# alexpreynolds/starch3

Hardware: AMD Instinct MI355X
Metric: input BED MB/s (cfg2, bzip2 -9, archive bit-identical to CPU starch3 path) (higher is better)
Workload: dtype u8

## Files before the change

starch_amd/csrc/bz2_bwt.hip:

```cpp
#include <string.h>
#include "bz2_int.hpp"
#include "bz2_bwt.hpp"

namespace bz {

constexpr int BT = 1024;
constexpr int NWV = BT / 64;

struct RadixSmem {
    uint32_t hist[256];
    uint32_t base[256];
    uint32_t wcnt[NWV][256];
    uint32_t scan[NWV + 1];
    uint32_t flag;
};

__device__ __forceinline__ uint64_t lanemask_lt()
{
    const int lane = threadIdx.x & 63;
    return lane ? (~0ull >> (64 - lane)) : 0ull;
}

template <class V>
__device__ bool radix_pass(const uint64_t* Ks, const V* Vs, uint64_t* Kd, V* Vd, uint32_t m, int shift,
// ... 713 lines not shown
                    slo[sp] = blo; shi[sp] = bhi; ++sp;
                }
                fbw_sync();
                continue;
            }
            const int32_t lo = cmd[1], hi = cmd[2], m = hi - lo + 1;
            for (int32_t q = lane; q < m; q += 64) { sk[q] = key[lo + q]; sf[q] = fmap[lo + q]; }
            __builtin_amdgcn_fence(__ATOMIC_RELEASE, "wavefront");
            __builtin_amdgcn_wave_barrier();
            __builtin_amdgcn_fence(__ATOMIC_ACQUIRE, "wavefront");
            if (lane == 0) fbp_qsort3(sk, sf, 0, m - 1, lcg);
            __builtin_amdgcn_fence(__ATOMIC_RELEASE, "wavefront");
            __builtin_amdgcn_wave_barrier();
            __builtin_amdgcn_fence(__ATOMIC_ACQUIRE, "wavefront");
            for (int32_t q = lane; q < m; q += 64) { key[lo + q] = sk[q]; fmap[lo + q] = sf[q]; }
            __builtin_amdgcn_fence(__ATOMIC_RELEASE, "wavefront");
            __builtin_amdgcn_wave_barrier();
            __builtin_amdgcn_fence(__ATOMIC_ACQUIRE, "wavefront");
        }
    }
}

__global__ void k_fb_heads(const uint32_t* __restrict__ key, const uint64_t* __restrict__ hp,
                           const uint32_t* __restrict__ mixed, uint32_t* __restrict__ head, uint32_t n, uint32_t stamp)
{
    const uint32_t i = blockIdx.x * blockDim.x + threadIdx.x;
    if (i == 0 || i >= n || head[i]) return;
    if (mixed[(uint32_t)hp[i]] == stamp && key[i] != key[i - 1]) head[i] = 1;
}

__global__ void k_fb_origptr(const uint32_t* __restrict__ fmap, BlockDesc* __restrict__ blocks, uint32_t b, uint32_t n)
{
    const uint32_t i = blockIdx.x * blockDim.x + threadIdx.x;
    if (i < n && fmap[i] == 0) blocks[b].orig_ptr = i;
}

void launch_bwt(BlockDesc* blocks, uint32_t b0, uint32_t nb, const uint8_t* blkbytes, uint64_t stride,
                const BwtScratch& scr, unsigned long long* stats, hipStream_t st)
{
    hipLaunchKernelGGL(k_bwt, dim3(nb), dim3(BT), 0, st, blocks, b0, blkbytes, stride, scr, stats);
    HIP_CHECK(hipGetLastError());
}

void FbPool::init(int device)
{
    if (dev == device) return;
    if (dev >= 0) throw StarchError(-10, "FbPool: device changed");
    for (int i = 0; i < kStreams; ++i) HIP_CHECK(hipStreamCreateWithFlags(&st[i], hipStreamNonBlocking));
    for (int i = 0; i <= kStreams; ++i) HIP_CHECK(hipEventCreateWithFlags(&ev[i], hipEventDisableTiming));
    dev = device;
}

FbPool::~FbPool()
{
    for (int i = 0; i < kStreams; ++i)
        if (st[i]) { (void)hipStreamSynchronize(st[i]); (void)hipStreamDestroy(st[i]); }
    for (int i = 0; i <= kStreams; ++i)
        if (ev[i]) (void)hipEventDestroy(ev[i]);
}

void launch_fallback(BlockDesc* blocks, uint32_t b0, const uint32_t* which_host, const uint32_t* n_host,
                     uint32_t nwhich, const uint8_t* blkbytes, uint64_t stride, const BwtScratch& scr, FbPool& pool,
                     hipStream_t st)
{
    int dev = 0, ncu = 256;
    HIP_CHECK(hipGetDevice(&dev));
    hipDeviceProp_t prop;
// ... 104 lines not shown
```

starch_amd/csrc/bz2_bwt3.hip:

```cpp
#include "bz2_int.hpp"
#include "bz2_bwt.hpp"

#include <algorithm>
#include <type_traits>

namespace bz {
namespace {

constexpr int PT = 256;
constexpr int PTILE = 32768;
constexpr int PDIG = 12;
constexpr int PNB = 1 << PDIG;
constexpr int PNB_WIDE = 8192;
static_assert(PTILE <= 32768 && PNB_WIDE <= 8192, "k3_scatter_lds packs (digit << 15) | rotation-in-tile");
constexpr int MAXT = (900064 + PTILE - 1) / PTILE;
constexpr uint32_t W_MAX = 64, S1_MAX = 128, S_MAX = 256, M0_MAX = 512, M1_MAX = 1024, M2_MAX = 2048, M3_MAX = 4096;
#ifndef STARCH_L_MIN
#define STARCH_L_MIN 4096
#endif
constexpr uint32_t L_MIN = STARCH_L_MIN;
constexpr uint32_t GB_MIN = 16384;
constexpr uint32_t GB_MAXN = 8192;
constexpr uint32_t HG_MIN_PUSH = 32768;
constexpr uint32_t RBITS = 20;
// ... 259 lines not shown
    if (tid < 256) {
        uint32_t c = tid, below = 0;
        for (uint32_t j = 0; j < (c >> 5); ++j) below += __popc(bd.in_use[j]);
        below += __popc(bd.in_use[c >> 5] & ((1u << (c & 31)) - 1u));
        sym[c] = (uint8_t)below;
    }
    uint32_t nin = 0;
    for (int j = 0; j < 8; ++j) nin += __popc(bd.in_use[j]);
    *nin_out = nin;
}

__device__ __forceinline__ uint32_t wg_pop(const Ctx& c, const uint32_t* qs, uint32_t* job_sh, uint32_t x)
{
    if (threadIdx.x == 0) *job_sh = xq_pop(c.qhead, qs, x);
    __syncthreads();
    const uint32_t j = *job_sh;
    __syncthreads();
    return j;
}

__device__ __forceinline__ uint32_t wave_pop(const Ctx& c, const uint32_t* qs, uint32_t x)
{
    uint32_t j = 0;
    if ((threadIdx.x & 63) == 0) j = xq_pop(c.qhead, qs, x);
    return (uint32_t)__shfl((int)j, 0, 64);
}

__device__ __forceinline__ void load_qsizes_binned(const Ctx& c, uint32_t* qs)
{
    if (threadIdx.x < 8) qs[threadIdx.x] = c.qseg[threadIdx.x + 1] - c.qseg[threadIdx.x];
    __syncthreads();
}

__global__ void __launch_bounds__(256) k3_pss(Ctx c)
{
    __shared__ uint8_t sym[256];
    const uint32_t slot = blockIdx.y, b = c.b0 + slot;
    const uint32_t n = c.blocks[b].n;
    uint32_t nin;
    load_sym(c.blocks[b], sym, &nin);
    const uint32_t B = nin > 1 ? (uint32_t)bits_for3(nin - 1) : 1u;
    const uint32_t nw = (uint32_t)(((uint64_t)(n + 128) * B + 63) / 64 + 1);
    if (blockIdx.x == 0 && threadIdx.x == 0) {
        Geo g;
        g.B = B;
        g.D = 64 / B;
        g.KB = g.D * B;
        g.Dp = (64 - PDIG) / B;
        g.nin = nin;
        g.D1 = (c.nbins == PNB_WIDE && B == 5 && nin <= 20) ? 3u : 0u;
        g.SH = g.D1 ? 3 * B : PDIG;
        g.pad = 0;
        c.L.geo[slot] = g;
        c.blocks[b].n_in_use = nin;
    }
    __syncthreads();
    const uint32_t w = blockIdx.x * 256 + threadIdx.x;
    if (w >= nw) return;
    const uint8_t* blk = c.blkbytes + (uint64_t)b * c.stride;
    const uint64_t bit0 = (uint64_t)w * 64;
    const uint64_t j0 = bit0 / B, j1 = (bit0 + 63) / B;
    uint64_t word = 0;
    if (B == 4 && j1 < n) {
        const uint4 v = *reinterpret_cast<const uint4*>(blk + j0);
        const uint32_t q[4] = {v.x, v.y, v.z, v.w};
#pragma unroll
        for (int k = 0; k < 16; ++k) word = (word << 4) | sym[(q[k >> 2] >> (8 * (k & 3))) & 0xffu];
        c.scr.K[(uint64_t)slot * c.scr.stride + w] = word;
        return;
    }
    for (uint64_t j = j0; j <= j1; ++j) {
        const uint64_t s = sym[blk[j < n ? j : j % n]];
        const int sh = 64 - (int)B - (int)(j * B - bit0);
        word |= sh >= 0 ? (s << sh) : (s >> (-sh));
    }
    c.scr.K[(uint64_t)slot * c.scr.stride + w] = word;
}

__device__ __forceinline__ uint32_t* tile_hist(const Ctx& c, uint32_t slot)
{
    return reinterpret_cast<uint32_t*>(c.scr.K + (uint64_t)slot * c.scr.stride + pss_words(c.scr.stride));
}

template <int NB>
__global__ void __launch_bounds__(PT) k3_hist(Ctx c)
{
    __shared__ uint32_t cnt[NB];
    const uint32_t slot = blockIdx.y, b = c.b0 + slot, tile = blockIdx.x;
    const uint32_t n = c.blocks[b].n;
    const uint32_t t0 = tile * PTILE;
    if (t0 >= n) return;
    const Geo geo = c.L.geo[slot];
    const uint32_t B = geo.B;
    const uint64_t* pss = c.scr.K + (uint64_t)slot * c.scr.stride;
    for (int i = threadIdx.x; i < NB; i += PT) cnt[i] = 0;
    __syncthreads();
    const uint32_t e = n - t0 < (uint32_t)PTILE ? n - t0 : (uint32_t)PTILE;
    for (uint32_t k0 = threadIdx.x * 16u; k0 < e; k0 += PT * 16u) {
        const uint64_t bit0 = (uint64_t)(t0 + k0) * B;
        const uint64_t q0 = bit0 >> 6;
        const uint32_t p0 = (uint32_t)(bit0 & 63u);
        const uint64_t w[4] = {pss[q0], pss[q0 + 1], pss[q0 + 2], pss[q0 + 3]};
#pragma unroll
        for (int k = 0; k < 16; ++k) {
            const uint32_t bit = p0 + (uint32_t)k * B;
            const uint32_t ix = bit >> 6, p = bit & 63u;
            const uint64_t a = ix == 0 ? w[0] : ix == 1 ? w[1] : w[2];
            const uint64_t nx = ix == 0 ? w[1] : ix == 1 ? w[2] : w[3];
            const uint64_t v = (a << p) | ((nx >> 1) >> (63u - p));
            if (k0 + k < e) atomicAdd(&cnt[top_digit(v, geo)], 1u);
        }
    }
    __syncthreads();
    uint32_t* th = tile_hist(c, slot) + (uint64_t)tile * NB;
    for (int i = threadIdx.x; i < NB; i += PT) th[i] = cnt[i];
}

constexpr int ST = 1024;

template <int NB>
__global__ void __launch_bounds__(ST) k3_scan(Ctx c)
{
    constexpr int Q = NB / (4 * ST);
    __shared__ uint32_t scan_sh[ST / 64 + 1];
    __shared__ uint32_t cls_sh[16];
    const int tid = threadIdx.x;
    const uint32_t slot = blockIdx.x, b = c.b0 + slot;
    const uint32_t n = c.blocks[b].n;
    const uint32_t ntile = (n + PTILE - 1) / PTILE;
    uint4* th = reinterpret_cast<uint4*>(tile_hist(c, slot));
    uint4* tot = th + (uint64_t)MAXT * (NB / 4);
    uint4 a[Q];
#pragma unroll
    for (int j = 0; j < Q; ++j) a[j] = make_uint4(0, 0, 0, 0);
#pragma unroll 4
    for (uint32_t k = 0; k < ntile; ++k) {
#pragma unroll
        for (int j = 0; j < Q; ++j) {
            const uint4 x = th[(uint64_t)k * (NB / 4) + tid * Q + j];
            a[j].x += x.x; a[j].y += x.y; a[j].z += x.z; a[j].w += x.w;
        }
    }
    uint32_t sum = 0;
#pragma unroll
// ... 2394 lines not shown
            }
            if (n0) {
                bin(c.L.m0, n0, bout);
                hipLaunchKernelGGL((k3_sort_lds<4, 2, D>), gm0, dim3(256), 0, st, c, bout, nullptr);
            }
            if (n1) {
                bin(c.L.m1, n1, bout);
                hipLaunchKernelGGL((k3_sort_lds<4, 4, D>), gm1, dim3(256), 0, st, c, bout, nullptr);
            }
            if (ns) {
                bin(c.L.s, ns, bout);
                clear_h();
                hipLaunchKernelGGL((k3_sort_grp<1, 2, D>), gs, dim3(256), 0, st, c, bout, c.L.s);
                hipLaunchKernelGGL((k3_sort_lds<1, 2, D>), dim3(ncu / 2), dim3(256), 0, st, c, c.L.s, hard_n);
            }
            if (ns2) {
                bin(c.L.s2, ns2, bout);
                clear_h();
                hipLaunchKernelGGL((k3_sort_grp<1, 4, D>), gs2, dim3(256), 0, st, c, bout, c.L.s2);
                hipLaunchKernelGGL((k3_sort_lds<1, 4, D>), dim3(ncu / 2), dim3(256), 0, st, c, c.L.s2, hard_n);
            }
            if (nw) {
                bin(c.L.w, nw, bout);
                hipLaunchKernelGGL(k3_sort_w<D>, gw, dim3(256), 0, st, c, bout);
            }
        };
        if (c.keysrc) leaf(std::true_type{});
        else leaf(std::false_type{});
        HIP_CHECK(hipGetLastError());
        zero((0x3Full << C_W) | bit(C_M0));
    };

    {
        const uint32_t maxw = (uint32_t)pss_words(scr.stride);
        hipLaunchKernelGGL(k3_pss, dim3((maxw + 255) / 256, nb), dim3(256), 0, st, c);
        if (wide) {
            hipLaunchKernelGGL(k3_hist<PNB_WIDE>, dim3(MAXT, nb), dim3(PT), 0, st, c);
            hipLaunchKernelGGL(k3_scan<PNB_WIDE>, dim3(nb), dim3(ST), 0, st, c);
        } else {
            hipLaunchKernelGGL(k3_hist<PNB>, dim3(MAXT, nb), dim3(PT), 0, st, c);
            hipLaunchKernelGGL(k3_scan<PNB>, dim3(nb), dim3(ST), 0, st, c);
        }
        uint32_t* head;
        uint32_t* seg;
        next_q(head, seg);
        c.qhead = head;
        c.qseg = nullptr;
        const dim3 gsc((ncu + 7) / 8 * 8);
        c.sdig = 1;
        if (wide) hipLaunchKernelGGL(k3_scatter_lds<PNB_WIDE>, gsc, dim3(SCT), 0, st, c);
        else hipLaunchKernelGGL(k3_scatter_lds<PNB>, gsc, dim3(SCT), 0, st, c);
        HIP_CHECK(hipGetLastError());
    }
    sort_groups();
    c.sdig = 0;
    uint32_t rtext = 0;
    uint64_t prev_tied = ~0ull;
    bool done = false;
    for (;;) {
        read_ctr();
        const uint32_t nt = hctr[C_T0 + c.tsel];
        const uint64_t tied = hctr[C_TS0 + c.tsel];
        if (nt == 0) { done = true; break; }
        if (rtext == TEXT_ROUNDS || (rtext > 0 && 2 * tied > prev_tied)) break;
        prev_tied = tied;
        ++rtext;
        c.rtext = rtext;
        const uint32_t cur = c.tsel;
        c.tsel ^= 1u;
        zero(bit(C_T0 + c.tsel) | bit(C_TS0 + c.tsel));
        hipLaunchKernelGGL(k3_classify_text, dim3((nt + 256 * CT_IPT - 1) / (256 * CT_IPT)), dim3(256), 0, st, c,
                           c.L.t[cur], nt);
        HIP_CHECK(hipGetLastError());
// ... 37 lines not shown
```

starch_amd/csrc/bz2_mtf.hip:

```cpp
#include "bz2_bwt.hpp"

namespace bz {

constexpr int MT = 1024;
constexpr int NCH_BIG = 256;
constexpr uint32_t LINE = 128;

__device__ __forceinline__ uint32_t nsym_run(uint32_t z) { return z ? (31 - __clz(z + 1)) : 0; }

struct RunSum {
    uint32_t nz;
    uint32_t lz;
    uint32_t tz;
    uint32_t inner;
};

__device__ __forceinline__ RunSum run_compose(const RunSum& a, const RunSum& b)
{
    RunSum r;
    if (!a.nz) {
        r.nz = b.nz; r.lz = a.lz + b.lz; r.tz = b.tz; r.inner = b.inner;
    } else if (!b.nz) {
        r.nz = 1; r.lz = a.lz; r.tz = a.tz + b.lz; r.inner = a.inner;
    } else {
// ... 70 lines not shown
        }
        ++o;
    }
    __device__ __forceinline__ void flush()
    {
        const uint32_t k = o & 15u;
        if (!k) return;
        const uint32_t w = o - k, p = s > w ? s - w : 0u;
        const uint32_t sh = 8u * (16u - k);
        const uint64_t rl = sh >= 64 ? hi >> (sh - 64) : ((lo >> sh) | (sh ? hi << (64 - sh) : 0ull));
        const uint64_t rh = sh >= 64 ? 0ull : hi >> sh;
        store_range(w, p, k, rl, rh);
    }
};

__device__ __forceinline__ void put_run(Out8& out, uint32_t z)
{
    while (z) {
        const uint32_t d = ((z - 1) & 1u) ? 1u : 0u;
        out.put(d);
        z = (z - (d + 1)) >> 1;
    }
}

constexpr uint32_t MCS = 512;
constexpr int MCT = 256;
constexpr int MST = 1024;

struct NibP {
    using State = NibState;
    using List = uint64_t;
    static constexpr uint32_t LO = 1, HI = 16;
    static constexpr uint32_t SW = 2, LW = 1;
    static constexpr uint32_t IXB = 4;
#ifndef STARCH_NIB_SIX
#define STARCH_NIB_SIX 0
#endif
    static constexpr bool SIX = STARCH_NIB_SIX != 0;
    __device__ static State empty() { State r; r.list = 0; r.set = 0; r.cnt = 0; return r; }
    __device__ static void add(State& st, uint32_t s)
    {
        if (!((st.set >> s) & 1u)) { st.set |= 1u << s; st.list |= (uint64_t)s << (4 * st.cnt); ++st.cnt; }
    }
    __device__ static State compose(const State& c, const State& d) { return nib_compose(c, d); }
    __device__ static State identity(uint32_t nin)
    {
        State st;
        st.list = 0;
        for (uint32_t i = 0; i < nin; ++i) st.list |= (uint64_t)i << (4 * i);
        st.set = nin >= 32 ? ~0u : (1u << nin) - 1u;
        st.cnt = nin;
        return st;
    }
    __device__ static List list_of(const State& st) { return st.list; }
    __device__ static uint32_t mtf(List& L, uint32_t s) { return nib_mtf(L, s); }
};

struct ByteState {
    uint64_t w[4];
    uint32_t set;
    uint32_t cnt;
};
struct ByteList { uint64_t w[4]; };

template <int NW>
struct ByteP {
    static_assert(NW == 3 || NW == 4, "ByteP: 3 or 4 list words");
    using State = ByteState;
    using List = ByteList;
    static constexpr uint32_t LO = NW == 3 ? 17 : 25, HI = NW == 3 ? 24 : 30;
    static constexpr uint32_t SW = 5, LW = 4;
    static constexpr uint32_t IXB = 8;
#ifndef STARCH_BYTE_SIX
#define STARCH_BYTE_SIX 0
#endif
    static constexpr bool SIX = STARCH_BYTE_SIX != 0;
    __device__ static void put(uint64_t* w, uint32_t i, uint32_t s)
    {
        const uint32_t j = i >> 3, sh = 8 * (i & 7);
#pragma unroll
        for (uint32_t q = 0; q < 4; ++q)
            if (q == j) w[q] = (w[q] & ~(0xFFull << sh)) | ((uint64_t)s << sh);
    }
    __device__ static uint32_t get(const uint64_t* w, uint32_t i)
    {
        const uint32_t j = i >> 3;
        const uint64_t x = j == 0 ? w[0] : j == 1 ? w[1] : j == 2 ? w[2] : w[3];
        return (uint32_t)(x >> (8 * (i & 7))) & 0xFFu;
    }
    __device__ static State empty()
    {
        State r;
        r.w[0] = r.w[1] = r.w[2] = r.w[3] = ~0ull;
        r.set = 0;
        r.cnt = 0;
        return r;
    }
    __device__ static void add(State& st, uint32_t s)
    {
        if (!((st.set >> s) & 1u)) { st.set |= 1u << s; put(st.w, st.cnt, s); ++st.cnt; }
    }
    __device__ static State compose(const State& c, const State& d)
    {
        State r = d;
        for (uint32_t i = 0; i < c.cnt; ++i) {
            const uint32_t sym = get(c.w, i);
            if (!((d.set >> sym) & 1u)) { put(r.w, r.cnt, sym); ++r.cnt; }
        }
        r.set = c.set | d.set;
// ... 17 lines not shown
    {
        const uint64_t pat = (uint64_t)s * 0x0101010101010101ull;
        uint64_t z[4] = {0, 0, 0, 0};
#pragma unroll
        for (int j = 0; j < NW; ++j) {
            const uint64_t x = L.w[j] ^ pat;
            z[j] = (x - 0x0101010101010101ull) & ~x & 0x8080808080808080ull;
        }
        const uint32_t k = z[0] ? ((uint32_t)__builtin_ctzll(z[0]) >> 3)
                         : z[1] ? 8u + ((uint32_t)__builtin_ctzll(z[1]) >> 3)
                         : (NW == 3 || z[2]) ? 16u + ((uint32_t)__builtin_ctzll(z[2]) >> 3)
                                : 24u + ((uint32_t)__builtin_ctzll(z[3]) >> 3);
        const uint32_t jk = k >> 3, kb = k & 7u;
        const uint64_t m = kb == 7u ? ~0ull : ((1ull << (8u * kb + 8u)) - 1ull);
        uint64_t carry = s;
#pragma unroll
        for (uint32_t j = 0; j < (uint32_t)NW; ++j) {
            const uint64_t nv = (L.w[j] << 8) | carry;
            carry = L.w[j] >> 56;
            L.w[j] = j < jk ? nv : (j == jk ? ((nv & m) | (L.w[j] & ~m)) : L.w[j]);
        }
        return k;
    }
};

template <class P>
struct MtfScr {
    uint64_t* base;
    uint32_t C;
    __device__ typename P::State* st() const { return reinterpret_cast<typename P::State*>(base); }
    __device__ typename P::List* l0() const { return reinterpret_cast<typename P::List*>(base + (uint64_t)P::SW * C); }
    __device__ RunSum* rs() const { return reinterpret_cast<RunSum*>(base + (uint64_t)(P::SW + P::LW) * C); }
    __device__ uint2* zo() const { return reinterpret_cast<uint2*>(base + (uint64_t)(P::SW + P::LW + 2) * C); }
    __device__ uint8_t* ix() const { return reinterpret_cast<uint8_t*>(base + (uint64_t)(P::SW + P::LW + 3) * C); }
};

template <class P>
__device__ __forceinline__ MtfScr<P> mtf_scr(uint64_t* K, uint64_t kstride, uint32_t slot, uint32_t C)
{
    MtfScr<P> m;
    m.base = K + (uint64_t)slot * kstride;
    m.C = C;
    return m;
}

template <class P>
__device__ __forceinline__ bool mtf_mine(uint32_t nin) { return nin >= P::LO && nin <= P::HI; }

template <class F>
__device__ __forceinline__ void visit_chunk(const uint8_t* ll, uint32_t a, uint32_t e, F&& f)
{
    const uint4* q = reinterpret_cast<const uint4*>(ll + a);
    const uint32_t np = (e - a + 15) / 16;
    uint4 cur = q[0];
#pragma unroll 1
    for (uint32_t i = 0; i < np; ++i) {
        const uint4 nxt = q[i + 1 < np ? i + 1 : i];
        const uint32_t lim = e - a - 16 * i;
        if (lim >= 16) {
            auto all = [&](int, uint32_t s) { f(s); };
            piece<true>(cur, 0, all);
        } else {
            auto some = [&](int k, uint32_t s) { if ((uint32_t)k < lim) f(s); };
            piece<true>(cur, 0, some);
        }
        cur = nxt;
    }
}

template <class F>
__device__ __forceinline__ void visit_chunk_lines(const uint8_t* ll, uint32_t a, uint32_t e, F&& f)
{
    const uint32_t full = a + ((e - a) & ~(LINE - 1));
#pragma unroll 1
    for (uint32_t j0 = a; j0 < full; j0 += LINE) visit_line<true>(ll + j0, [&](int, uint32_t s) { f(s); });
    if (full < e) {
        const uint32_t lim = e - full;
        visit_line<true>(ll + full, [&](int k, uint32_t s) { if ((uint32_t)k < lim) f(s); });
    }
}

template <class P>
__global__ void __launch_bounds__(MCT) k_mtf_local(const BlockDesc* __restrict__ blocks, uint32_t b0,
                                                   const uint8_t* __restrict__ LL, uint64_t ll_stride,
                                                   uint64_t* __restrict__ K, uint64_t kstride, uint32_t C, uint32_t cs)
{
    const uint32_t slot = blockIdx.y, b = b0 + slot;
    const uint32_t n = blocks[b].n, nin = blocks[b].n_in_use;
    const uint32_t ch = blockIdx.x * MCT + threadIdx.x;
    const uint32_t a = ch * cs;
    if (!mtf_mine<P>(nin) || a >= n) return;
    const uint32_t e = a + cs < n ? a + cs : n;
    const uint8_t* ll = LL + (uint64_t)slot * ll_stride;
    typename P::State loc = P::empty();
    const uint32_t full = a + ((e - a) & ~(LINE - 1));
    auto add = [&](uint32_t s) { P::add(loc, s); };
    if (full < e) {
        const uint32_t lim = e - full;
        visit_line<false>(ll + full, [&](int k, uint32_t s) { if ((uint32_t)k < lim) add(s); });
    }
#pragma unroll 1
    for (uint32_t j0 = full; j0 > a && loc.cnt < nin;) {
        j0 -= LINE;
        visit_line<false>(ll + j0, [&](int, uint32_t s) { add(s); });
    }
    mtf_scr<P>(K, kstride, slot, C).st()[ch] = loc;
}

template <class P>
__global__ void __launch_bounds__(MST) k_mtf_scan_lists(const BlockDesc* __restrict__ blocks, uint32_t b0,
                                                        uint64_t* __restrict__ K, uint64_t kstride, uint32_t C,
                                                        uint32_t cs)
{
    __shared__ typename P::State sh[MST];
    const int tid = threadIdx.x;
    const uint32_t slot = blockIdx.x, b = b0 + slot;
    const uint32_t n = blocks[b].n, nin = blocks[b].n_in_use;
    if (!mtf_mine<P>(nin)) return;
    const uint32_t nch = (n + cs - 1) / cs;
    const uint32_t per = (nch + MST - 1) / MST;
    const MtfScr<P> ms = mtf_scr<P>(K, kstride, slot, C);
    const uint32_t c0 = tid * per;
    typename P::State agg = P::empty();
    for (uint32_t q = 0; q < per; ++q)
        if (c0 + q < nch) agg = P::compose(agg, ms.st()[c0 + q]);
    sh[tid] = agg;
    __syncthreads();
    for (int d = 1; d < MST; d <<= 1) {
        const typename P::State v = (tid >= d) ? P::compose(sh[tid - d], sh[tid]) : sh[tid];
        __syncthreads();
        sh[tid] = v;
        __syncthreads();
    }
    typename P::State st = P::identity(nin);
    if (tid) st = P::compose(st, sh[tid - 1]);
    for (uint32_t q = 0; q < per; ++q) {
        if (c0 + q >= nch) break;
        ms.l0()[c0 + q] = P::list_of(st);
        st = P::compose(st, ms.st()[c0 + q]);
    }
}

template <class P>
__global__ void __launch_bounds__(MCT) k_mtf_runs(const BlockDesc* __restrict__ blocks, uint32_t b0,
                                                  const uint8_t* __restrict__ LL, uint64_t ll_stride,
                                                  uint64_t* __restrict__ K, uint64_t kstride, uint32_t C, uint32_t cs)
{
    const uint32_t slot = blockIdx.y, b = b0 + slot;
    const uint32_t n = blocks[b].n, nin = blocks[b].n_in_use;
    const uint32_t ch = blockIdx.x * MCT + threadIdx.x;
    const uint32_t a = ch * cs;
    if (!mtf_mine<P>(nin) || a >= n) return;
    const uint32_t e = a + cs < n ? a + cs : n;
    const MtfScr<P> ms = mtf_scr<P>(K, kstride, slot, C);
    uint32_t z = 0, nz = 0, lz = 0, inner = 0;
    if constexpr (!P::SIX) {
        const uint8_t* ll = LL + (uint64_t)slot * ll_stride;
        uint32_t prev = a ? ll[a - 1] : 0u;
        visit_chunk_lines(ll, a, e, [&](uint32_t s) {
            const uint32_t nzf = s != prev ? 1u : 0u;
            prev = s;
            inner += (nzf & nz) ? 1u + (31u - __clz(z + 1u)) : 0u;
            lz = (nzf & (nz ^ 1u)) ? z : lz;
            nz |= nzf;
            z = nzf ? 0u : z + 1u;
        });
        RunSum r;
        r.nz = nz;
        r.lz = nz ? lz : z;
        r.tz = nz ? z : 0u;
        r.inner = inner;
        ms.rs()[ch] = r;
        return;
    }
    typename P::List L = ms.l0()[ch];
    uint8_t* ixp = ms.ix() + (uint64_t)a * P::IXB / 8;
    uint64_t lo = 0, hi = 0;
    uint32_t k16 = 0, piece_no = 0;
    visit_chunk(LL + (uint64_t)slot * ll_stride, a, e, [&](uint32_t s) {
        const uint32_t x = P::mtf(L, s);
        if constexpr (P::IXB == 4) {
            lo = (lo >> 4) | ((uint64_t)x << 60);
        } else {
            lo = (lo >> 8) | (hi << 56);
            hi = (hi >> 8) | ((uint64_t)x << 56);
        }
        if (P::SIX && ++k16 == 16) {
            if constexpr (P::IXB == 4) reinterpret_cast<uint64_t*>(ixp)[piece_no] = lo;
            else reinterpret_cast<uint4*>(ixp)[piece_no] = make_uint4((uint32_t)lo, (uint32_t)(lo >> 32),
                                                                      (uint32_t)hi, (uint32_t)(hi >> 32));
            k16 = 0;
            ++piece_no;
        }
        const uint32_t nzf = x != 0 ? 1u : 0u;
        inner += (nzf & nz) ? 1u + (31u - __clz(z + 1u)) : 0u;
        lz = (nzf & (nz ^ 1u)) ? z : lz;
        nz |= nzf;
        z = nzf ? 0u : z + 1u;
    });
    if (P::SIX && k16) {
        const uint32_t sh = (16 - k16) * P::IXB;
        if constexpr (P::IXB == 4) {
            reinterpret_cast<uint64_t*>(ixp)[piece_no] = lo >> sh;
        } else {
            const uint64_t l2 = sh >= 64 ? hi >> (sh - 64) : ((lo >> sh) | (hi << (64 - sh)));
            const uint64_t h2 = sh >= 64 ? 0 : hi >> sh;
            reinterpret_cast<uint4*>(ixp)[piece_no] = make_uint4((uint32_t)l2, (uint32_t)(l2 >> 32), (uint32_t)h2,
                                                                 (uint32_t)(h2 >> 32));
        }
    }
    RunSum r;
    r.nz = nz;
    r.lz = nz ? lz : z;
    r.tz = nz ? z : 0u;
    r.inner = inner;
    ms.rs()[ch] = r;
}

template <class P>
__global__ void __launch_bounds__(MST) k_mtf_scan_runs(BlockDesc* __restrict__ blocks, uint32_t b0,
                                                       uint64_t* __restrict__ K, uint64_t kstride, uint32_t C,
                                                       uint32_t cs, uint16_t* __restrict__ mtfv_all, uint64_t mtf_stride)
{
    __shared__ RunSum sh[MST];
    const int tid = threadIdx.x;
    const uint32_t slot = blockIdx.x, b = b0 + slot;
    const uint32_t n = blocks[b].n, nin = blocks[b].n_in_use;
    if (!mtf_mine<P>(nin)) return;
    const uint32_t nch = (n + cs - 1) / cs;
    const uint32_t per = (nch + MST - 1) / MST;
    const MtfScr<P> ms = mtf_scr<P>(K, kstride, slot, C);
    const uint32_t c0 = tid * per;
    RunSum agg;
    agg.nz = 0; agg.lz = 0; agg.tz = 0; agg.inner = 0;
    for (uint32_t q = 0; q < per; ++q)
        if (c0 + q < nch) agg = run_compose(agg, ms.rs()[c0 + q]);
    sh[tid] = agg;
    __syncthreads();
    for (int d = 1; d < MST; d <<= 1) {
        const RunSum v = (tid >= d) ? run_compose(sh[tid - d], sh[tid]) : sh[tid];
        __syncthreads();
        sh[tid] = v;
        __syncthreads();
    }
    RunSum ex;
    ex.nz = 0; ex.lz = 0; ex.tz = 0; ex.inner = 0;
    if (tid) ex = sh[tid - 1];
    for (uint32_t q = 0; q < per; ++q) {
        if (c0 + q >= nch) break;
        const uint32_t zin = ex.nz ? ex.tz : ex.lz;
        const uint32_t obase = ex.nz ? nsym_run(ex.lz) + 1 + ex.inner : 0;
        ms.zo()[c0 + q] = make_uint2(zin, obase);
        ex = run_compose(ex, ms.rs()[c0 + q]);
    }
    if (tid == MST - 1) {
        const RunSum T = sh[MST - 1];
        uint8_t* mtfv = reinterpret_cast<uint8_t*>(mtfv_all + (uint64_t)b * mtf_stride);
        uint32_t z = T.nz ? T.tz : T.lz;
        uint32_t o = T.nz ? nsym_run(T.lz) + 1 + T.inner : 0;
        while (z) {
            const uint32_t d = ((z - 1) & 1u) ? 1u : 0u;
            mtfv[o++] = (uint8_t)d;
            z = (z - (d + 1)) >> 1;
        }
        mtfv[o++] = (uint8_t)(nin + 1);
        blocks[b].n_mtf = o;
    }
}

template <class P>
__global__ void __launch_bounds__(MCT) k_mtf_emit(const BlockDesc* __restrict__ blocks, uint32_t b0,
                                                  const uint8_t* __restrict__ LL, uint64_t ll_stride,
                                                  const uint64_t* __restrict__ K, uint64_t kstride, uint32_t C,
                                                  uint32_t cs, uint16_t* __restrict__ mtfv_all, uint64_t mtf_stride)
{
    const uint32_t slot = blockIdx.y, b = b0 + slot;
    const uint32_t n = blocks[b].n, nin = blocks[b].n_in_use;
    const uint32_t ch = blockIdx.x * MCT + threadIdx.x;
    const uint32_t a = ch * cs;
    if (!mtf_mine<P>(nin) || a >= n) return;
    const uint32_t e = a + cs < n ? a + cs : n;
    const MtfScr<P> ms = mtf_scr<P>(const_cast<uint64_t*>(K), kstride, slot, C);
    const uint2 zo = ms.zo()[ch];
    Out8 out;
    out.init(reinterpret_cast<uint8_t*>(mtfv_all + (uint64_t)b * mtf_stride), zo.y);
    uint32_t z = zo.x;
    auto f = [&](uint32_t x) {
        if (x == 0) {
            ++z;
        } else {
            put_run(out, z);
            out.put(x + 1);
            z = 0;
        }
    };
    if constexpr (!P::SIX) {
        typename P::List L = ms.l0()[ch];
        visit_chunk_lines(LL + (uint64_t)slot * ll_stride, a, e, [&](uint32_t s) { f(P::mtf(L, s)); });
        out.flush();
        return;
    }
    constexpr uint32_t SPP = 128 / P::IXB;
    const uint4* q = reinterpret_cast<const uint4*>(ms.ix() + (uint64_t)a * P::IXB / 8);
    const uint32_t cnt = e - a, np = (cnt + SPP - 1) / SPP;
    uint4 cur = q[0];
#pragma unroll 1
    for (uint32_t i = 0; i < np; ++i) {
        const uint4 nxt = q[i + 1 < np ? i + 1 : i];
        const uint32_t wv[4] = {cur.x, cur.y, cur.z, cur.w};
        const uint32_t lim = cnt - i * SPP;
        if (lim >= SPP) {
#pragma unroll
            for (uint32_t k = 0; k < SPP; ++k)
                f(P::IXB == 4 ? (wv[k >> 3] >> (4 * (k & 7))) & 15u : (wv[k >> 2] >> (8 * (k & 3))) & 255u);
        } else {
#pragma unroll
            for (uint32_t k = 0; k < SPP; ++k)
                if (k < lim) f(P::IXB == 4 ? (wv[k >> 3] >> (4 * (k & 7))) & 15u : (wv[k >> 2] >> (8 * (k & 3))) & 255u);
        }
        cur = nxt;
    }
    out.flush();
}

__global__ void __launch_bounds__(MT) k_mtf_big(BlockDesc* __restrict__ blocks, uint32_t b0,
                                                 const uint8_t* __restrict__ LL, uint64_t ll_stride,
                                                 uint8_t* __restrict__ scratch, uint64_t scratch_stride,
                                                 uint16_t* __restrict__ mtfv_all, uint64_t mtf_stride,
                                                 Tables* __restrict__ tabs)
{
    constexpr uint32_t C = NCH_BIG;
    constexpr int NF = 4;
    __shared__ RunSum cs_sh[C];
    __shared__ uint32_t freq[NF][258];
    __shared__ uint32_t scan_sh[MT / 64 + 1];
    __shared__ uint32_t tail[2];
    __shared__ uint8_t lst[256 * NCH_BIG];
    __shared__ uint32_t seen[NCH_BIG][8];
    __shared__ uint8_t st[256], st2[256], fl[256];
    __shared__ uint32_t lcnt[NCH_BIG];
    __shared__ uint32_t zin_sh[C], out_sh[C];

    const int tid = threadIdx.x;
    const uint32_t slot = blockIdx.x;
    const uint32_t b = b0 + slot;
    const uint32_t n = blocks[b].n;
    const uint32_t nin = blocks[b].n_in_use;
    if (nin <= ByteP<4>::HI) return;
    for (int i = tid; i < NF * 258; i += MT) (&freq[0][0])[i] = 0;
    const uint8_t* ll = LL + (uint64_t)slot * ll_stride;
    uint8_t* idx = scratch + (uint64_t)slot * scratch_stride;
    uint8_t* locl = idx + ((n + 255u) & ~255u);
    uint8_t* sstate = locl + 256ull * C;
    uint16_t* mtfv = mtfv_all + (uint64_t)b * mtf_stride;
// ... 149 lines not shown
        for (int t = 0; t < 16; ++t) w[t >> 2] |= (uint32_t)seq[blk[p[t] ? p[t] - 1 : n - 1]] << (8 * (t & 3));
        *reinterpret_cast<uint4*>(scr.LL + so + j) = make_uint4(w[0], w[1], w[2], w[3]);
    } else {
        for (uint32_t t = j; t < n; ++t) {
            const uint32_t pp = scr.SA[so + t];
            scr.LL[so + t] = seq[blk[pp ? pp - 1 : n - 1]];
        }
    }
}

void launch_last_col(const BlockDesc* blocks, uint32_t b0, const uint32_t* which, uint32_t nwhich,
                     const uint8_t* blkbytes, uint64_t stride, const BwtScratch& scr, hipStream_t st)
{
    if (!nwhich) return;
    const uint32_t ntile = (uint32_t)((scr.stride + LC_TILE - 1) / LC_TILE);
    const uint32_t grid = ntile * ((nwhich + 7) / 8 * 8);
    hipLaunchKernelGGL(k_last_col, dim3(grid), dim3(256), 0, st, blocks, b0, which, nwhich, ntile, blkbytes, stride,
                       scr);
    HIP_CHECK(hipGetLastError());
}

void launch_mtf(BlockDesc* blocks, uint32_t b0, uint32_t nb, const uint8_t* blkbytes, uint64_t stride,
                const BwtScratch& scr, uint16_t* mtfv, uint64_t mtf_stride, Tables* tabs, hipStream_t st,
                uint32_t need)
{
    (void)blkbytes;
    (void)stride;
    const uint32_t cs = nb >= 256 ? MCS : nb >= 64 ? 256u : nb >= 8 ? 128u : 64u;
    const uint32_t C = (uint32_t)((scr.stride + cs - 1) / cs);
    const uint64_t kstride = scr.stride;
    const dim3 gch((C + MCT - 1) / MCT, nb);
    auto run = [&](auto pol) {
        using P = decltype(pol);
        hipLaunchKernelGGL(k_mtf_local<P>, gch, dim3(MCT), 0, st, blocks, b0, scr.LL, scr.stride, scr.K, kstride, C, cs);
        hipLaunchKernelGGL(k_mtf_scan_lists<P>, dim3(nb), dim3(MST), 0, st, blocks, b0, scr.K, kstride, C, cs);
        hipLaunchKernelGGL(k_mtf_runs<P>, gch, dim3(MCT), 0, st, blocks, b0, scr.LL, scr.stride, scr.K, kstride, C,
                           cs);
        hipLaunchKernelGGL(k_mtf_scan_runs<P>, dim3(nb), dim3(MST), 0, st, blocks, b0, scr.K, kstride, C, cs, mtfv,
                           mtf_stride);
        hipLaunchKernelGGL(k_mtf_emit<P>, gch, dim3(MCT), 0, st, blocks, b0, scr.LL, scr.stride, scr.K, kstride, C,
                           cs, mtfv, mtf_stride);
    };
    if (need & kMtfNib) run(NibP{});
    if (need & kMtfByte3) run(ByteP<3>{});
    if (need & kMtfByte4) run(ByteP<4>{});
    if (need & kMtfBig)
        hipLaunchKernelGGL(k_mtf_big, dim3(nb), dim3(MT), 0, st, blocks, b0, scr.LL, scr.stride,
                           reinterpret_cast<uint8_t*>(scr.K), scr.stride * sizeof(uint64_t), mtfv, mtf_stride, tabs);
    HIP_CHECK(hipGetLastError());
}

}
```

Measured before the change: 86010.

## Fuse PSS packing with tile histogram, merge MTF pre/scan kernels, tweak origptr

Packing the symbol stream into PSS words now happens inside the tile-histogram kernel. Each thread builds a group of 64 symbols in registers, writes the packed words and counts digits directly, so the hist kernel no longer re-reads PSS from global memory and one launch is removed. In MTF, the local-list pass and the run-summary pass become one pre-kernel, and the two scan kernels become one, which cuts passes over the last column and kernel launches. The unused SIX index-packing path is removed. It also changes orig_ptr to 0 for single-symbol blocks of at least 10000 bytes, apparently to match the CPU reference's main-sort behaviour, which is a correctness change.

```diff
diff --git a/starch_amd/csrc/bz2_bwt.hip b/starch_amd/csrc/bz2_bwt.hip
--- a/starch_amd/csrc/bz2_bwt.hip
+++ b/starch_amd/csrc/bz2_bwt.hip
@@ -769,7 +769,8 @@
 __global__ void k_fb_origptr(const uint32_t* __restrict__ fmap, BlockDesc* __restrict__ blocks, uint32_t b, uint32_t n)
 {
     const uint32_t i = blockIdx.x * blockDim.x + threadIdx.x;
-    if (i < n && fmap[i] == 0) blocks[b].orig_ptr = i;
+    const bool main_sorted = blocks[b].n_in_use == 1 && n >= 10000;
+    if (i < n && fmap[i] == 0) blocks[b].orig_ptr = main_sorted ? 0u : i;
 }
 
 void launch_bwt(BlockDesc* blocks, uint32_t b0, uint32_t nb, const uint8_t* blkbytes, uint64_t stride,
diff --git a/starch_amd/csrc/bz2_bwt3.hip b/starch_amd/csrc/bz2_bwt3.hip
--- a/starch_amd/csrc/bz2_bwt3.hip
+++ b/starch_amd/csrc/bz2_bwt3.hip
@@ -315,84 +315,125 @@
     __syncthreads();
 }
 
-__global__ void __launch_bounds__(256) k3_pss(Ctx c)
-{
+__device__ __forceinline__ uint32_t* tile_hist(const Ctx& c, uint32_t slot)
+{
+    return reinterpret_cast<uint32_t*>(c.scr.K + (uint64_t)slot * c.scr.stride + pss_words(c.scr.stride));
+}
+
+constexpr uint32_t PGRP = 64;
+static_assert(PTILE % PGRP == 0, "tiles own whole groups, groups own whole PSS words");
+
+template <int B>
+__device__ __forceinline__ void pss_hist_group(const uint8_t* __restrict__ blk, const uint8_t* sym, uint32_t n,
+                                               uint32_t g, uint32_t nw, uint64_t* __restrict__ pss, uint32_t* cnt,
+                                               Geo geo)
+{
+    constexpr int NTAIL = (16 + B - 1) / B;
+    constexpr int NRAW = (int)(PGRP + 16) / 4;
+    static_assert(NTAIL <= 16, "the tail symbols come from one more 16-byte load");
+    const uint32_t j0 = g * PGRP;
+    uint32_t raw[NRAW];
+    if (j0 + PGRP + 16 <= n) {
+        const uint4* q = reinterpret_cast<const uint4*>(blk + j0);
+        const uint4 v0 = q[0], v1 = q[1], v2 = q[2], v3 = q[3], v4 = q[4];
+        raw[0] = v0.x; raw[1] = v0.y; raw[2] = v0.z; raw[3] = v0.w;
+        raw[4] = v1.x; raw[5] = v1.y; raw[6] = v1.z; raw[7] = v1.w;
+        raw[8] = v2.x; raw[9] = v2.y; raw[10] = v2.z; raw[11] = v2.w;
+        raw[12] = v3.x; raw[13] = v3.y; raw[14] = v3.z; raw[15] = v3.w;
+        raw[16] = v4.x; raw[17] = v4.y; raw[18] = v4.z; raw[19] = v4.w;
+    } else {
+        uint32_t jj = j0 < n ? j0 : j0 % n;
+#pragma unroll
+        for (int i = 0; i < NRAW; ++i) {
+            uint32_t x = 0;
+#pragma unroll
+            for (int t = 0; t < 4; ++t) {
+                if (4 * i + t < (int)PGRP + NTAIL) {
+                    x |= (uint32_t)blk[jj] << (8 * t);
+                    jj = jj + 1 == n ? 0u : jj + 1;
+                }
+            }
+            raw[i] = x;
+        }
+    }
+    uint64_t w[B + 1];
+#pragma unroll
+    for (int i = 0; i <= B; ++i) w[i] = 0;
+#pragma unroll
+    for (int k = 0; k < (int)PGRP + NTAIL; ++k) {
+        const uint64_t sy = sym[(raw[k >> 2] >> (8 * (k & 3))) & 0xffu];
+        const int bit = k * B, ix = bit >> 6, sh = 64 - B - (bit & 63);
+        if (sh >= 0) {
+            w[ix] |= sy << sh;
+        } else {
+            w[ix] |= sy >> (-sh);
+            if (ix < B) w[ix + 1] |= sy << (64 + sh);
+        }
+    }
+    const uint32_t w0 = g * B;
+    if (w0 + B <= nw) {
+#pragma unroll
+        for (int i = 0; i < B; ++i) pss[w0 + i] = w[i];
+    } else {
+#pragma unroll
+        for (int i = 0; i < B; ++i)
+            if (w0 + i < nw) pss[w0 + i] = w[i];
+    }
+    if (j0 >= n) return;
+    geo.B = B;
+#pragma unroll
+    for (int k = 0; k < (int)PGRP; ++k) {
+        const int bit = k * B, ix = bit >> 6, p = bit & 63;
+        const uint64_t v = (w[ix] << p) | ((w[ix + 1] >> 1) >> (63 - p));
+        if (j0 + k < n) atomicAdd(&cnt[top_digit(v, geo)], 1u);
+    }
+}
+
+template <int NB>
+__global__ void __launch_bounds__(PT) k3_pss_hist(Ctx c)
+{
+    __shared__ uint32_t cnt[NB];
     __shared__ uint8_t sym[256];
-    const uint32_t slot = blockIdx.y, b = c.b0 + slot;
+    const uint32_t slot = blockIdx.y, b = c.b0 + slot, tile = blockIdx.x;
     const uint32_t n = c.blocks[b].n;
     uint32_t nin;
     load_sym(c.blocks[b], sym, &nin);
-    const uint32_t B = nin > 1 ? (uint32_t)bits_for3(nin - 1) : 1u;
-    const uint32_t nw = (uint32_t)(((uint64_t)(n + 128) * B + 63) / 64 + 1);
-    if (blockIdx.x == 0 && threadIdx.x == 0) {
-        Geo g;
-        g.B = B;
-        g.D = 64 / B;
-        g.KB = g.D * B;
-        g.Dp = (64 - PDIG) / B;
-        g.nin = nin;
-        g.D1 = (c.nbins == PNB_WIDE && B == 5 && nin <= 20) ? 3u : 0u;
-        g.SH = g.D1 ? 3 * B : PDIG;
-        g.pad = 0;
-        c.L.geo[slot] = g;
+    Geo geo;
+    geo.B = nin > 1 ? (uint32_t)bits_for3(nin - 1) : 1u;
+    geo.D = 64 / geo.B;
+    geo.KB = geo.D * geo.B;
+    geo.Dp = (64 - PDIG) / geo.B;
+    geo.nin = nin;
+    geo.D1 = (c.nbins == PNB_WIDE && geo.B == 5 && nin <= 20) ? 3u : 0u;
+    geo.SH = geo.D1 ? 3 * geo.B : PDIG;
+    geo.pad = 0;
+    if (tile == 0 && threadIdx.x == 0) {
+        c.L.geo[slot] = geo;
         c.blocks[b].n_in_use = nin;
     }
-    __syncthreads();
-    const uint32_t w = blockIdx.x * 256 + threadIdx.x;
-    if (w >= nw) return;
-    const uint8_t* blk = c.blkbytes + (uint64_t)b * c.stride;
-    const uint64_t bit0 = (uint64_t)w * 64;
-    const uint64_t j0 = bit0 / B, j1 = (bit0 + 63) / B;
-    uint64_t word = 0;
-    if (B == 4 && j1 < n) {
-        const uint4 v = *reinterpret_cast<const uint4*>(blk + j0);
-        const uint32_t q[4] = {v.x, v.y, v.z, v.w};
-#pragma unroll
-        for (int k = 0; k < 16; ++k) word = (word << 4) | sym[(q[k >> 2] >> (8 * (k & 3))) & 0xffu];
-        c.scr.K[(uint64_t)slot * c.scr.stride + w] = word;
-        return;
-    }
-    for (uint64_t j = j0; j <= j1; ++j) {
-        const uint64_t s = sym[blk[j < n ? j : j % n]];
-        const int sh = 64 - (int)B - (int)(j * B - bit0);
-        word |= sh >= 0 ? (s << sh) : (s >> (-sh));
-    }
-    c.scr.K[(uint64_t)slot * c.scr.stride + w] = word;
-}
-
-__device__ __forceinline__ uint32_t* tile_hist(const Ctx& c, uint32_t slot)
-{
-    return reinterpret_cast<uint32_t*>(c.scr.K + (uint64_t)slot * c.scr.stride + pss_words(c.scr.stride));
-}
-
-template <int NB>
-__global__ void __launch_bounds__(PT) k3_hist(Ctx c)
-{
-    __shared__ uint32_t cnt[NB];
-    const uint32_t slot = blockIdx.y, b = c.b0 + slot, tile = blockIdx.x;
-    const uint32_t n = c.blocks[b].n;
     const uint32_t t0 = tile * PTILE;
     if (t0 >= n) return;
-    const Geo geo = c.L.geo[slot];
-    const uint32_t B = geo.B;
-    const uint64_t* pss = c.scr.K + (uint64_t)slot * c.scr.stride;
     for (int i = threadIdx.x; i < NB; i += PT) cnt[i] = 0;
     __syncthreads();
-    const uint32_t e = n - t0 < (uint32_t)PTILE ? n - t0 : (uint32_t)PTILE;
-    for (uint32_t k0 = threadIdx.x * 16u; k0 < e; k0 += PT * 16u) {
-        const uint64_t bit0 = (uint64_t)(t0 + k0) * B;
-        const uint64_t q0 = bit0 >> 6;
-        const uint32_t p0 = (uint32_t)(bit0 & 63u);
-        const uint64_t w[4] = {pss[q0], pss[q0 + 1], pss[q0 + 2], pss[q0 + 3]};
-#pragma unroll
-        for (int k = 0; k < 16; ++k) {
-            const uint32_t bit = p0 + (uint32_t)k * B;
-            const uint32_t ix = bit >> 6, p = bit & 63u;
-            const uint64_t a = ix == 0 ? w[0] : ix == 1 ? w[1] : w[2];
-            const uint64_t nx = ix == 0 ? w[1] : ix == 1 ? w[2] : w[3];
-            const uint64_t v = (a << p) | ((nx >> 1) >> (63u - p));
-            if (k0 + k < e) atomicAdd(&cnt[top_digit(v, geo)], 1u);
-        }
+    const uint32_t B = geo.B;
+    const uint32_t nw = (uint32_t)(((uint64_t)(n + 128) * B + 63) / 64 + 1);
+    const uint32_t g0 = tile * (PTILE / PGRP);
+    const uint32_t g1 = n - t0 <= (uint32_t)PTILE ? (nw + B - 1) / B : g0 + PTILE / PGRP;
+    const uint8_t* blk = c.blkbytes + (uint64_t)b * c.stride;
+    uint64_t* pss = c.scr.K + (uint64_t)slot * c.scr.stride;
+    auto run = [&](auto bc) {
+        for (uint32_t g = g0 + threadIdx.x; g < g1; g += PT)
+            pss_hist_group<decltype(bc)::value>(blk, sym, n, g, nw, pss, cnt, geo);
+    };
+    switch (B) {
+    case 1: run(std::integral_constant<int, 1>{}); break;
+    case 2: run(std::integral_constant<int, 2>{}); break;
+    case 3: run(std::integral_constant<int, 3>{}); break;
+    case 4: run(std::integral_constant<int, 4>{}); break;
+    case 5: run(std::integral_constant<int, 5>{}); break;
+    case 6: run(std::integral_constant<int, 6>{}); break;
+    case 7: run(std::integral_constant<int, 7>{}); break;
+    default: run(std::integral_constant<int, 8>{}); break;
     }
     __syncthreads();
     uint32_t* th = tile_hist(c, slot) + (uint64_t)tile * NB;
@@ -2853,13 +2894,11 @@
     };
 
     {
-        const uint32_t maxw = (uint32_t)pss_words(scr.stride);
-        hipLaunchKernelGGL(k3_pss, dim3((maxw + 255) / 256, nb), dim3(256), 0, st, c);
         if (wide) {
-            hipLaunchKernelGGL(k3_hist<PNB_WIDE>, dim3(MAXT, nb), dim3(PT), 0, st, c);
+            hipLaunchKernelGGL(k3_pss_hist<PNB_WIDE>, dim3(MAXT, nb), dim3(PT), 0, st, c);
             hipLaunchKernelGGL(k3_scan<PNB_WIDE>, dim3(nb), dim3(ST), 0, st, c);
         } else {
-            hipLaunchKernelGGL(k3_hist<PNB>, dim3(MAXT, nb), dim3(PT), 0, st, c);
+            hipLaunchKernelGGL(k3_pss_hist<PNB>, dim3(MAXT, nb), dim3(PT), 0, st, c);
             hipLaunchKernelGGL(k3_scan<PNB>, dim3(nb), dim3(ST), 0, st, c);
         }
         uint32_t* head;
diff --git a/starch_amd/csrc/bz2_mtf.hip b/starch_amd/csrc/bz2_mtf.hip
--- a/starch_amd/csrc/bz2_mtf.hip
+++ b/starch_amd/csrc/bz2_mtf.hip
@@ -126,11 +126,6 @@
     using List = uint64_t;
     static constexpr uint32_t LO = 1, HI = 16;
     static constexpr uint32_t SW = 2, LW = 1;
-    static constexpr uint32_t IXB = 4;
-#ifndef STARCH_NIB_SIX
-#define STARCH_NIB_SIX 0
-#endif
-    static constexpr bool SIX = STARCH_NIB_SIX != 0;
     __device__ static State empty() { State r; r.list = 0; r.set = 0; r.cnt = 0; return r; }
     __device__ static void add(State& st, uint32_t s)
     {
@@ -164,11 +159,6 @@
     using List = ByteList;
     static constexpr uint32_t LO = NW == 3 ? 17 : 25, HI = NW == 3 ? 24 : 30;
     static constexpr uint32_t SW = 5, LW = 4;
-    static constexpr uint32_t IXB = 8;
-#ifndef STARCH_BYTE_SIX
-#define STARCH_BYTE_SIX 0
-#endif
-    static constexpr bool SIX = STARCH_BYTE_SIX != 0;
     __device__ static void put(uint64_t* w, uint32_t i, uint32_t s)
     {
         const uint32_t j = i >> 3, sh = 8 * (i & 7);
@@ -252,7 +242,6 @@
     __device__ typename P::List* l0() const { return reinterpret_cast<typename P::List*>(base + (uint64_t)P::SW * C); }
     __device__ RunSum* rs() const { return reinterpret_cast<RunSum*>(base + (uint64_t)(P::SW + P::LW) * C); }
     __device__ uint2* zo() const { return reinterpret_cast<uint2*>(base + (uint64_t)(P::SW + P::LW + 2) * C); }
-    __device__ uint8_t* ix() const { return reinterpret_cast<uint8_t*>(base + (uint64_t)(P::SW + P::LW + 3) * C); }
 };
 
 template <class P>
@@ -266,27 +255,6 @@
 
 template <class P>
 __device__ __forceinline__ bool mtf_mine(uint32_t nin) { return nin >= P::LO && nin <= P::HI; }
-
-template <class F>
-__device__ __forceinline__ void visit_chunk(const uint8_t* ll, uint32_t a, uint32_t e, F&& f)
-{
-    const uint4* q = reinterpret_cast<const uint4*>(ll + a);
-    const uint32_t np = (e - a + 15) / 16;
-    uint4 cur = q[0];
-#pragma unroll 1
-    for (uint32_t i = 0; i < np; ++i) {
-        const uint4 nxt = q[i + 1 < np ? i + 1 : i];
-        const uint32_t lim = e - a - 16 * i;
-        if (lim >= 16) {
-            auto all = [&](int, uint32_t s) { f(s); };
-            piece<true>(cur, 0, all);
-        } else {
-            auto some = [&](int k, uint32_t s) { if ((uint32_t)k < lim) f(s); };
-            piece<true>(cur, 0, some);
-        }
-        cur = nxt;
-    }
-}
 
 template <class F>
 __device__ __forceinline__ void visit_chunk_lines(const uint8_t* ll, uint32_t a, uint32_t e, F&& f)
@@ -301,9 +269,9 @@
 }
 
 template <class P>
-__global__ void __launch_bounds__(MCT) k_mtf_local(const BlockDesc* __restrict__ blocks, uint32_t b0,
-                                                   const uint8_t* __restrict__ LL, uint64_t ll_stride,
-                                                   uint64_t* __restrict__ K, uint64_t kstride, uint32_t C, uint32_t cs)
+__global__ void __launch_bounds__(MCT) k_mtf_pre(const BlockDesc* __restrict__ blocks, uint32_t b0,
+                                                 const uint8_t* __restrict__ LL, uint64_t ll_stride,
+                                                 uint64_t* __restrict__ K, uint64_t kstride, uint32_t C, uint32_t cs)
 {
     const uint32_t slot = blockIdx.y, b = b0 + slot;
     const uint32_t n = blocks[b].n, nin = blocks[b].n_in_use;
@@ -312,6 +280,23 @@
     if (!mtf_mine<P>(nin) || a >= n) return;
     const uint32_t e = a + cs < n ? a + cs : n;
     const uint8_t* ll = LL + (uint64_t)slot * ll_stride;
+    const MtfScr<P> ms = mtf_scr<P>(K, kstride, slot, C);
+    uint32_t z = 0, nz = 0, lz = 0, inner = 0;
+    uint32_t prev = a ? ll[a - 1] : 0u;
+    visit_chunk_lines(ll, a, e, [&](uint32_t s) {
+        const uint32_t nzf = s != prev ? 1u : 0u;
+        prev = s;
+        inner += (nzf & nz) ? 1u + (31u - __clz(z + 1u)) : 0u;
+        lz = (nzf & (nz ^ 1u)) ? z : lz;
+        nz |= nzf;
+        z = nzf ? 0u : z + 1u;
+    });
+    RunSum r;
+    r.nz = nz;
+    r.lz = nz ? lz : z;
+    r.tz = nz ? z : 0u;
+    r.inner = inner;
+    ms.rs()[ch] = r;
     typename P::State loc = P::empty();
     const uint32_t full = a + ((e - a) & ~(LINE - 1));
     auto add = [&](uint32_t s) { P::add(loc, s); };
@@ -324,15 +309,16 @@
         j0 -= LINE;
         visit_line<false>(ll + j0, [&](int, uint32_t s) { add(s); });
     }
-    mtf_scr<P>(K, kstride, slot, C).st()[ch] = loc;
+    ms.st()[ch] = loc;
 }
 
 template <class P>
-__global__ void __launch_bounds__(MST) k_mtf_scan_lists(const BlockDesc* __restrict__ blocks, uint32_t b0,
-                                                        uint64_t* __restrict__ K, uint64_t kstride, uint32_t C,
-                                                        uint32_t cs)
+__global__ void __launch_bounds__(MST) k_mtf_scan(BlockDesc* __restrict__ blocks, uint32_t b0,
+                                                  uint64_t* __restrict__ K, uint64_t kstride, uint32_t C, uint32_t cs,
+                                                  uint16_t* __restrict__ mtfv_all, uint64_t mtf_stride)
 {
     __shared__ typename P::State sh[MST];
+    __shared__ RunSum shr[MST];
     const int tid = threadIdx.x;
     const uint32_t slot = blockIdx.x, b = b0 + slot;
     const uint32_t n = blocks[b].n, nin = blocks[b].n_in_use;
@@ -342,139 +328,42 @@
     const MtfScr<P> ms = mtf_scr<P>(K, kstride, slot, C);
     const uint32_t c0 = tid * per;
     typename P::State agg = P::empty();
+    RunSum ragg;
+    ragg.nz = 0; ragg.lz = 0; ragg.tz = 0; ragg.inner = 0;
     for (uint32_t q = 0; q < per; ++q)
-        if (c0 + q < nch) agg = P::compose(agg, ms.st()[c0 + q]);
+        if (c0 + q < nch) {
+            agg = P::compose(agg, ms.st()[c0 + q]);
+            ragg = run_compose(ragg, ms.rs()[c0 + q]);
+        }
     sh[tid] = agg;
+    shr[tid] = ragg;
     __syncthreads();
     for (int d = 1; d < MST; d <<= 1) {
         const typename P::State v = (tid >= d) ? P::compose(sh[tid - d], sh[tid]) : sh[tid];
+        const RunSum rv = (tid >= d) ? run_compose(shr[tid - d], shr[tid]) : shr[tid];
         __syncthreads();
         sh[tid] = v;
+        shr[tid] = rv;
         __syncthreads();
     }
     typename P::State st = P::identity(nin);
-    if (tid) st = P::compose(st, sh[tid - 1]);
+    RunSum ex;
+    ex.nz = 0; ex.lz = 0; ex.tz = 0; ex.inner = 0;
+    if (tid) {
+        st = P::compose(st, sh[tid - 1]);
+        ex = shr[tid - 1];
+    }
     for (uint32_t q = 0; q < per; ++q) {
         if (c0 + q >= nch) break;
         ms.l0()[c0 + q] = P::list_of(st);
         st = P::compose(st, ms.st()[c0 + q]);
-    }
-}
-
-template <class P>
-__global__ void __launch_bounds__(MCT) k_mtf_runs(const BlockDesc* __restrict__ blocks, uint32_t b0,
-                                                  const uint8_t* __restrict__ LL, uint64_t ll_stride,
-                                                  uint64_t* __restrict__ K, uint64_t kstride, uint32_t C, uint32_t cs)
-{
-    const uint32_t slot = blockIdx.y, b = b0 + slot;
-    const uint32_t n = blocks[b].n, nin = blocks[b].n_in_use;
-    const uint32_t ch = blockIdx.x * MCT + threadIdx.x;
-    const uint32_t a = ch * cs;
-    if (!mtf_mine<P>(nin) || a >= n) return;
-    const uint32_t e = a + cs < n ? a + cs : n;
-    const MtfScr<P> ms = mtf_scr<P>(K, kstride, slot, C);
-    uint32_t z = 0, nz = 0, lz = 0, inner = 0;
-    if constexpr (!P::SIX) {
-        const uint8_t* ll = LL + (uint64_t)slot * ll_stride;
-        uint32_t prev = a ? ll[a - 1] : 0u;
-        visit_chunk_lines(ll, a, e, [&](uint32_t s) {
-            const uint32_t nzf = s != prev ? 1u : 0u;
-            prev = s;
-            inner += (nzf & nz) ? 1u + (31u - __clz(z + 1u)) : 0u;
-            lz = (nzf & (nz ^ 1u)) ? z : lz;
-            nz |= nzf;
-            z = nzf ? 0u : z + 1u;
-        });
-        RunSum r;
-        r.nz = nz;
-        r.lz = nz ? lz : z;
-        r.tz = nz ? z : 0u;
-        r.inner = inner;
-        ms.rs()[ch] = r;
-        return;
-    }
-    typename P::List L = ms.l0()[ch];
-    uint8_t* ixp = ms.ix() + (uint64_t)a * P::IXB / 8;
-    uint64_t lo = 0, hi = 0;
-    uint32_t k16 = 0, piece_no = 0;
-    visit_chunk(LL + (uint64_t)slot * ll_stride, a, e, [&](uint32_t s) {
-        const uint32_t x = P::mtf(L, s);
-        if constexpr (P::IXB == 4) {
-            lo = (lo >> 4) | ((uint64_t)x << 60);
-        } else {
-            lo = (lo >> 8) | (hi << 56);
-            hi = (hi >> 8) | ((uint64_t)x << 56);
-        }
-        if (P::SIX && ++k16 == 16) {
-            if constexpr (P::IXB == 4) reinterpret_cast<uint64_t*>(ixp)[piece_no] = lo;
-            else reinterpret_cast<uint4*>(ixp)[piece_no] = make_uint4((uint32_t)lo, (uint32_t)(lo >> 32),
-                                                                      (uint32_t)hi, (uint32_t)(hi >> 32));
-            k16 = 0;
-            ++piece_no;
-        }
-        const uint32_t nzf = x != 0 ? 1u : 0u;
-        inner += (nzf & nz) ? 1u + (31u - __clz(z + 1u)) : 0u;
-        lz = (nzf & (nz ^ 1u)) ? z : lz;
-        nz |= nzf;
-        z = nzf ? 0u : z + 1u;
-    });
-    if (P::SIX && k16) {
-        const uint32_t sh = (16 - k16) * P::IXB;
-        if constexpr (P::IXB == 4) {
-            reinterpret_cast<uint64_t*>(ixp)[piece_no] = lo >> sh;
-        } else {
-            const uint64_t l2 = sh >= 64 ? hi >> (sh - 64) : ((lo >> sh) | (hi << (64 - sh)));
-            const uint64_t h2 = sh >= 64 ? 0 : hi >> sh;
-            reinterpret_cast<uint4*>(ixp)[piece_no] = make_uint4((uint32_t)l2, (uint32_t)(l2 >> 32), (uint32_t)h2,
-                                                                 (uint32_t)(h2 >> 32));
-        }
-    }
-    RunSum r;
-    r.nz = nz;
-    r.lz = nz ? lz : z;
-    r.tz = nz ? z : 0u;
-    r.inner = inner;
-    ms.rs()[ch] = r;
-}
-
-template <class P>
-__global__ void __launch_bounds__(MST) k_mtf_scan_runs(BlockDesc* __restrict__ blocks, uint32_t b0,
-                                                       uint64_t* __restrict__ K, uint64_t kstride, uint32_t C,
-                                                       uint32_t cs, uint16_t* __restrict__ mtfv_all, uint64_t mtf_stride)
-{
-    __shared__ RunSum sh[MST];
-    const int tid = threadIdx.x;
-    const uint32_t slot = blockIdx.x, b = b0 + slot;
-    const uint32_t n = blocks[b].n, nin = blocks[b].n_in_use;
-    if (!mtf_mine<P>(nin)) return;
-    const uint32_t nch = (n + cs - 1) / cs;
-    const uint32_t per = (nch + MST - 1) / MST;
-    const MtfScr<P> ms = mtf_scr<P>(K, kstride, slot, C);
-    const uint32_t c0 = tid * per;
-    RunSum agg;
-    agg.nz = 0; agg.lz = 0; agg.tz = 0; agg.inner = 0;
-    for (uint32_t q = 0; q < per; ++q)
-        if (c0 + q < nch) agg = run_compose(agg, ms.rs()[c0 + q]);
-    sh[tid] = agg;
-    __syncthreads();
-    for (int d = 1; d < MST; d <<= 1) {
-        const RunSum v = (tid >= d) ? run_compose(sh[tid - d], sh[tid]) : sh[tid];
-        __syncthreads();
-        sh[tid] = v;
-        __syncthreads();
-    }
-    RunSum ex;
-    ex.nz = 0; ex.lz = 0; ex.tz = 0; ex.inner = 0;
-    if (tid) ex = sh[tid - 1];
-    for (uint32_t q = 0; q < per; ++q) {
-        if (c0 + q >= nch) break;
         const uint32_t zin = ex.nz ? ex.tz : ex.lz;
         const uint32_t obase = ex.nz ? nsym_run(ex.lz) + 1 + ex.inner : 0;
         ms.zo()[c0 + q] = make_uint2(zin, obase);
         ex = run_compose(ex, ms.rs()[c0 + q]);
     }
     if (tid == MST - 1) {
-        const RunSum T = sh[MST - 1];
+        const RunSum T = shr[MST - 1];
         uint8_t* mtfv = reinterpret_cast<uint8_t*>(mtfv_all + (uint64_t)b * mtf_stride);
         uint32_t z = T.nz ? T.tz : T.lz;
         uint32_t o = T.nz ? nsym_run(T.lz) + 1 + T.inner : 0;
@@ -514,32 +403,8 @@
             z = 0;
         }
     };
-    if constexpr (!P::SIX) {
-        typename P::List L = ms.l0()[ch];
-        visit_chunk_lines(LL + (uint64_t)slot * ll_stride, a, e, [&](uint32_t s) { f(P::mtf(L, s)); });
-        out.flush();
-        return;
-    }
-    constexpr uint32_t SPP = 128 / P::IXB;
-    const uint4* q = reinterpret_cast<const uint4*>(ms.ix() + (uint64_t)a * P::IXB / 8);
-    const uint32_t cnt = e - a, np = (cnt + SPP - 1) / SPP;
-    uint4 cur = q[0];
-#pragma unroll 1
-    for (uint32_t i = 0; i < np; ++i) {
-        const uint4 nxt = q[i + 1 < np ? i + 1 : i];
-        const uint32_t wv[4] = {cur.x, cur.y, cur.z, cur.w};
-        const uint32_t lim = cnt - i * SPP;
-        if (lim >= SPP) {
-#pragma unroll
-            for (uint32_t k = 0; k < SPP; ++k)
-                f(P::IXB == 4 ? (wv[k >> 3] >> (4 * (k & 7))) & 15u : (wv[k >> 2] >> (8 * (k & 3))) & 255u);
-        } else {
-#pragma unroll
-            for (uint32_t k = 0; k < SPP; ++k)
-                if (k < lim) f(P::IXB == 4 ? (wv[k >> 3] >> (4 * (k & 7))) & 15u : (wv[k >> 2] >> (8 * (k & 3))) & 255u);
-        }
-        cur = nxt;
-    }
+    typename P::List L = ms.l0()[ch];
+    visit_chunk_lines(LL + (uint64_t)slot * ll_stride, a, e, [&](uint32_t s) { f(P::mtf(L, s)); });
     out.flush();
 }
 
@@ -755,11 +620,8 @@
     const dim3 gch((C + MCT - 1) / MCT, nb);
     auto run = [&](auto pol) {
         using P = decltype(pol);
-        hipLaunchKernelGGL(k_mtf_local<P>, gch, dim3(MCT), 0, st, blocks, b0, scr.LL, scr.stride, scr.K, kstride, C, cs);
-        hipLaunchKernelGGL(k_mtf_scan_lists<P>, dim3(nb), dim3(MST), 0, st, blocks, b0, scr.K, kstride, C, cs);
-        hipLaunchKernelGGL(k_mtf_runs<P>, gch, dim3(MCT), 0, st, blocks, b0, scr.LL, scr.stride, scr.K, kstride, C,
-                           cs);
-        hipLaunchKernelGGL(k_mtf_scan_runs<P>, dim3(nb), dim3(MST), 0, st, blocks, b0, scr.K, kstride, C, cs, mtfv,
+        hipLaunchKernelGGL(k_mtf_pre<P>, gch, dim3(MCT), 0, st, blocks, b0, scr.LL, scr.stride, scr.K, kstride, C, cs);
+        hipLaunchKernelGGL(k_mtf_scan<P>, dim3(nb), dim3(MST), 0, st, blocks, b0, scr.K, kstride, C, cs, mtfv,
                            mtf_stride);
         hipLaunchKernelGGL(k_mtf_emit<P>, gch, dim3(MCT), 0, st, blocks, b0, scr.LL, scr.stride, scr.K, kstride, C,
                            cs, mtfv, mtf_stride);
```

After: 87040 (median of 6 runs). 1.2% higher.
